# baycom/tfrec

Measured on AMD Instinct MI355X. Metric: IQ MSamples/s through demod+decode (batched streams), higher is better.
Workload: dtype int32+f32+f64

## Files before the change

### tfrec_amd/csrc/slicers.h

```cpp
#pragma once


struct Slicer {
	int lbi;
	int cur_block;
	int mark_lvl, rssi_i;
	int bitcnt, dmin, dmax, offset, last_bit;
	int first_cand_g;
	int td_lo, td_hi;
	int ib;
	int split;
	int hi, lo;
};
__device__ __forceinline__ void tfa2_thresholds(Slicer &f)
{
	const int noffset = d2i(0.9 * f.offset);
	f.hi = noffset + f.dmax / 32;
	f.lo = noffset + f.dmin / 32;
}

__device__ __forceinline__ void slicer_fresh(Slicer &f, int kind)
{
	f.mark_lvl = 0;
	f.rssi_i = 0;
	f.bitcnt = 0;
	f.dmin = 32767;
	f.dmax = -32767;
	f.offset = 0;
	f.last_bit = 0;
	f.first_cand_g = -1;
	f.hi = f.lo = 0;
	(void)kind;
}

__device__ __forceinline__ void slicer_chunk_begin(Slicer &f, int gf)
{
	const int b = gf >> 13;
	if (b != f.cur_block) {
		f.lbi = rebase_lbi(f.lbi, f.cur_block, b);
		f.cur_block = b;
	}
	const int o = gf & (kBlockDec - 1);
	f.ib = 2 * o;
	f.split = kBlockDec - o;
}
__device__ __forceinline__ int slicer_index(Slicer &f, int k)
{
	if (__builtin_expect(__ballot(k == f.split) != 0ull, 0)) {
		if (k == f.split) {
			f.lbi = rebase_lbi(f.lbi, f.cur_block, f.cur_block + 1);
			f.cur_block++;
			f.ib -= kIndexSpan;
		}
	}
	return f.ib + 2 * k;
}

__device__ __forceinline__ void tfa1_sample(Slicer &f, BitWriter &bw, int k, int I, int Q, int pI, int pQ)
{
	const int index = slicer_index(f, k);
	const int dev = fm_dev_nrzs(I, Q, pI, pQ);
	{
		const int decayed = tfa1_decay(f.mark_lvl);
		f.mark_lvl = dev > f.mark_lvl ? dev : decayed;
	}
	if (f.mark_lvl > f.rssi_i)
		f.rssi_i = f.mark_lvl;
	if (dev < (int)((uint32_t)f.mark_lvl >> 1)) {
		if (f.lbi) {
			const int gap = index - f.lbi;
			if (gap > 4) {
				for (int n = 22; n <= gap; n += 20)
					bw.put(1);
				bw.put(0);
			}
		}
		if (index - f.lbi > 2)
			f.lbi = index;
	}
}

__device__ __forceinline__ void tfa2_candidate(Slicer &f, BitWriter &bw, int g, int index, int bit, double spb, uint64_t nb_mul)
{
	if (f.first_cand_g < 0)
		f.first_cand_g = g;
	if (index > f.lbi + 8) {
		f.bitcnt++;
		const int tdiff = index - f.lbi;
		if (tdiff >= f.td_lo && tdiff <= f.td_hi) {
			const int numbits = nb_mul ? tfa2_numbits_mul(tdiff, nb_mul) : d2i(((tdiff / 2) + (spb / 2)) / spb);
			const int run = (numbits < 32 && numbits > 1) ? numbits - 1 : 0;
			bw.put_bits((f.last_bit ? (1u << run) - 1u : 0u) | ((uint32_t)bit << run), run + 1);
			f.last_bit = bit;
		}
	}
	if (index - f.lbi > 2)
		f.lbi = index;
}

__device__ __forceinline__ void tfa2_sample(Slicer &f, BitWriter &bw, int g, int k, int ld, uint32_t iq, double spb, uint64_t nb_mul)
{
	const int index = slicer_index(f, k);
	if (f.bitcnt < 10) {
		const bool up = ld > f.dmax, down = ld < f.dmin;
		if (up)
			f.dmax = (7 * f.dmax + ld) / 8;
		if (down)
			f.dmin = (7 * f.dmin + ld) / 8;
		if (up || down) {
			f.offset = (f.dmax + f.dmin) / 2;
			tfa2_thresholds(f);
		}
		if (f.bitcnt > 4) {
			const int I = (int)(int16_t)(iq & 0xffff), Q = (int)iq >> 16;
			const uint32_t t = (uint32_t)f.rssi_i + (uint32_t)(I * I) + (uint32_t)(Q * Q);
			f.rssi_i = (int)((uint32_t)f.rssi_i + (uint32_t)((int)t / 100));
		}
	}
	const int hi = f.hi, lo = f.lo;
	const int bit = ld > hi ? 1 : 0;
	if ((ld > hi || ld < lo) && bit != f.last_bit)
		tfa2_candidate(f, bw, g, index, bit, spb, nb_mul);
}

struct Slot8 {
	uint4 q0, q1, q2, q3, q4, q5, q6, q7;
};
struct Slot4 {
	uint4 q0, q1, q2, q3;
};

template <int KIND>
__device__ __forceinline__ int run_window(Slicer &f, BitWriter &bw, int g0, int last, bool closed,
					  const uint32_t *__restrict__ drow, const uint32_t *__restrict__ ldslots, int prevI,
					  int prevQ, double spb, uint64_t nb_mul, uint4 *__restrict__ my_lds, int head_chunks)
{
	const int n = last - g0 + 1;
	const int nch = (n + kChunk - 1) >> 5;
	if (KIND == 0) {
		auto load = [&](int i) -> Slot8 {
			const u32x4_a4 *p = reinterpret_cast<const u32x4_a4 *>(drow + g0 + kChunk * i);
			Slot8 r;
			u32x4_a4 v;
			v = p[0]; r.q0 = make_uint4(v.x, v.y, v.z, v.w);
			v = p[1]; r.q1 = make_uint4(v.x, v.y, v.z, v.w);
			v = p[2]; r.q2 = make_uint4(v.x, v.y, v.z, v.w);
			v = p[3]; r.q3 = make_uint4(v.x, v.y, v.z, v.w);
			v = p[4]; r.q4 = make_uint4(v.x, v.y, v.z, v.w);
			v = p[5]; r.q5 = make_uint4(v.x, v.y, v.z, v.w);
			v = p[6]; r.q6 = make_uint4(v.x, v.y, v.z, v.w);
			v = p[7]; r.q7 = make_uint4(v.x, v.y, v.z, v.w);
			return r;
		};
		int pI = prevI, pQ = prevQ;
		if (g0 > 0) {
			const uint32_t pw = drow[g0 - 1];
			pI = (int)(int16_t)(pw & 0xffff);
			pQ = (int)pw >> 16;
		}
		Slot8 cur = load(0);
		for (int i = 0; i < nch; i++) {
			my_lds[0 * 64] = cur.q0; my_lds[1 * 64] = cur.q1; my_lds[2 * 64] = cur.q2; my_lds[3 * 64] = cur.q3;
			my_lds[4 * 64] = cur.q4; my_lds[5 * 64] = cur.q5; my_lds[6 * 64] = cur.q6; my_lds[7 * 64] = cur.q7;
			const Slot8 nxt = load(i + 1 < nch ? i + 1 : i);
			const int nv = n - kChunk * i < kChunk ? n - kChunk * i : kChunk;
			slicer_chunk_begin(f, g0 + kChunk * i);
			uint4 vn = my_lds[0];
#pragma unroll 1
			for (int q = 0; 4 * q < nv; q++) {
				const uint4 v = vn;
				vn = my_lds[((q + 1) & 7) * 64];
				const uint32_t vw[4] = { v.x, v.y, v.z, v.w };
#pragma unroll
				for (int t = 0; t < 4; t++) {
					const int I = (int)(int16_t)(vw[t] & 0xffff), Q = (int)vw[t] >> 16;
					if (4 * q + t < nv)
						tfa1_sample(f, bw, 4 * q + t, I, Q, pI, pQ);
					pI = I;
					pQ = Q;
				}
			}
			bw.chunk_end();
			cur = nxt;
		}
	} else {
		auto load = [&](int i) -> Slot4 {
			const uint4 *p = reinterpret_cast<const uint4 *>(ldslots + (size_t)i * 16);
			Slot4 r;
			r.q0 = p[0]; r.q1 = p[1]; r.q2 = p[2]; r.q3 = p[3];
			return r;
		};
		Slot4 cur = load(0);
		for (int i = 0; i < nch; i++) {
			my_lds[0 * 64] = cur.q0; my_lds[1 * 64] = cur.q1; my_lds[2 * 64] = cur.q2; my_lds[3 * 64] = cur.q3;
			const Slot4 nxt = load(i + 1 < nch ? i + 1 : i);
			const int nv = n - kChunk * i < kChunk ? n - kChunk * i : kChunk;
			slicer_chunk_begin(f, g0 + kChunk * i);
			uint4 vn = my_lds[0];
#pragma unroll 1
			for (int q = 0; 8 * q < nv; q++) {
				const uint4 v = vn;
				vn = my_lds[((q + 1) & 3) * 64];
				const uint32_t vw[4] = { v.x, v.y, v.z, v.w };
#pragma unroll
				for (int t = 0; t < 8; t++) {
					if (8 * q + t < nv) {
						const int ld = (int)(int16_t)((vw[t >> 1] >> (16 * (t & 1))) & 0xffff);
						const uint32_t iq = (f.bitcnt > 4 && f.bitcnt < 10) ? drow[g0 + kChunk * i + 8 * q + t] : 0u;
						tfa2_sample(f, bw, g0 + kChunk * i + 8 * q + t, 8 * q + t, ld, iq, spb, nb_mul);
					}
				}
			}
			bw.chunk_end();
			cur = nxt;
			if (head_chunks > 0 && (f.bitcnt >= 10 || i + 1 >= head_chunks) && i + 1 < nch)
				return i + 1;
		}
	}
	const int bl = last >> 13;
	if (bl != f.cur_block) {
		f.lbi = rebase_lbi(f.lbi, f.cur_block, bl);
		f.cur_block = bl;
	}
	if (closed && KIND == 1)
		for (int q = 0; q < 16; q++)
			bw.put(f.last_bit);
	return nch;
}

template <int KIND>
__device__ __forceinline__ void window_task(int c, int j, int n_streams, int M, const uint32_t *__restrict__ dec,
					    size_t dec_stride, const int16_t *__restrict__ ld16, const ChainLaunch &L,
					    const WinTables &T, bool exact_lbi, int lbi_in_override, uint4 *__restrict__ my_lds,
					    int head_chunks)
{
	const int a = c / n_streams, s = c - a * n_streams;
	const ChainParams &p = L.params[a];
	const ChainState &st = L.states[a][s];
	const int og = T.open[(size_t)c * T.cap + j];
	const int close = T.close[(size_t)c * T.cap + j];
	const bool closed = close < M;
	const int last = closed ? close : M - 1;
	const bool cont = (j == 0) && T.cont[c];
	Slicer f;
	slicer_fresh(f, KIND);
	f.cur_block = og >> 13;
	if (cont) {
		f.mark_lvl = st.mark_lvl;
		f.rssi_i = st.rssi_i;
		f.bitcnt = st.bitcnt;
		f.dmin = st.dmin;
		f.dmax = st.dmax;
		f.offset = st.offset;
		f.last_bit = st.last_bit;
		f.lbi = rebase_lbi(st.last_bit_idx, -1, f.cur_block);
	} else if (KIND == 0) {
		f.lbi = 0;
	} else if (exact_lbi) {
		f.lbi = lbi_in_override;
	} else if (j == 0) {
		f.lbi = rebase_lbi(st.last_bit_idx, -1, f.cur_block);
	} else {
		f.lbi = kSpecLbi;
	}
	if (KIND == 1) {
		tfa2_thresholds(f);
		f.td_lo = (int)floor(p.spb / 4) + 1;
		f.td_hi = (int)ceil(32 * p.spb) - 1;
	}
	BitWriter bw{ T.bits + (size_t)c * T.bit_words + (og >> 6) + 3 * j, 0u, 0, 0u, -1 };
	const uint32_t *drow = dec + (size_t)s * dec_stride;
	const uint32_t *ldslots = (KIND == 1) ? reinterpret_cast<const uint32_t *>(ld16 + (size_t)(c - T.ld_c0) * T.slots * 32) +
							(size_t)win_slot0(og, j) * 16
					      : nullptr;
	const int resume = run_window<KIND>(f, bw, og, last, closed, drow, ldslots, st.prev_i, st.prev_q, p.spb, p.nb_mul, my_lds,
					    head_chunks);
	bw.finish();
	WinResult &r = T.result[(size_t)c * T.cap + j];
	r.resume = resume < ((last - og + 1 + kChunk - 1) >> 5) ? resume : -1;
	r.nbits = bw.n;
	r.closed = closed ? 1 : 0;
	r.rssi_i = f.rssi_i;
	r.offset = f.offset;
	r.lbi_out = f.lbi;
	r.first_cand_g = f.first_cand_g;
	r.bitcnt = f.bitcnt;
	r.dmin = f.dmin;
	r.dmax = f.dmax;
	r.last_bit = f.last_bit;
	r.mark_lvl = f.mark_lvl;
}

__global__ __launch_bounds__(64) void slicer_kernel(const uint32_t *__restrict__ dec, size_t dec_stride,
						    const int16_t *__restrict__ ld16, int n_streams, int n_blocks, ChainLaunch L,
						    WinTables T, int lanes, int head_chunks, int kind, int qsel)
{
	extern __shared__ uint4 slot_lds[];
	uint4 *my_lds = slot_lds + threadIdx.x;
	if ((int)threadIdx.x >= lanes)
		return;
	const int M = n_blocks * kBlockDec;
	const size_t total = (size_t)L.n_active * n_streams * T.cap;
	for (int q = 2 * kind + (kind == 0 ? 1 : 0); q < 2 * kind + 2; q++) {
		if ((qsel == 1 && (q & 1)) || (qsel == 2 && !(q & 1)))
			continue;
		const uint32_t count = T.queue[q].count;
		const int head = (q & 1) == 0 ? head_chunks : 0;
		while (true) {
			const uint32_t idx = atomicAdd(&T.queue[q].head, 1u);
			if (idx >= count)
				break;
			const uint2 it = T.items[(size_t)q * total + idx];
			const int c = (int)it.x, j = (int)it.y;
			if (kind == 0)
				window_task<0>(c, j, n_streams, M, dec, dec_stride, ld16, L, T, false, 0, my_lds, 0);
			else
				window_task<1>(c, j, n_streams, M, dec, dec_stride, ld16, L, T, false, 0, my_lds, head);
		}
	}
}

__global__ __launch_bounds__(256) void mark_kernel(const uint32_t *__restrict__ dec, size_t dec_stride, int n_streams,
						  int n_blocks, ChainLaunch L, WinTables T)
{
	const int M = n_blocks * kBlockDec;
	const size_t total = (size_t)L.n_active * n_streams * T.cap;
	const uint32_t count = T.queue[7].count;
	const uint32_t tid = blockIdx.x * 256 + threadIdx.x, nthreads = gridDim.x * 256;
	for (uint32_t idx = tid; idx < count; idx += nthreads) {
		const uint2 it = T.items[(size_t)7 * total + idx];
		const int c = (int)it.x, j = (int)(it.y & 0x1ffffu), pc = (int)(it.y >> 17);
		const int a = c / n_streams, s = c - a * n_streams;
		const ChainState &st = L.states[a][s];
		const int og = T.open[(size_t)c * T.cap + j];
		const int close = T.close[(size_t)c * T.cap + j];
		const int n = (close < M ? close : M - 1) - og + 1;
		const uint32_t *drow = dec + (size_t)s * dec_stride;
		const uint32_t prev0 = ((uint32_t)st.prev_i & 0xffffu) | ((uint32_t)st.prev_q << 16);
		const int slot0 = win_slot0(og, j);
		const int i0 = pc * kMarkSlots;
		const int nch = (n + 31) >> 5;
		const int i1 = nch < i0 + kMarkSlots ? nch : i0 + kMarkSlots;
		const int iw = pc == 0 ? 0 : i0 - kMarkWarmSlots;
		int mark = (pc == 0 && j == 0 && T.cont[c]) ? st.mark_lvl : 0;
		int start = mark, mx = 0;
		K3Chunk<true> A, B;
		k3_load<true>(A, drow, og + 32 * iw, prev0);
		for (int i = iw; i < i1; i++) {
			if (i + 1 < i1)
				k3_load<true>(B, drow, og + 32 * (i + 1), prev0);
			if (i == i0)
				start = mark;
			const int nv = n - 32 * i < 32 ? n - 32 * i : 32;
			int pI = (int)(int16_t)(A.prevw & 0xffff), pQ = (int)A.prevw >> 16;
			uint32_t bits = 0;
			if (__ballot(nv < 32) == 0ull) {
				uint32_t rev = 0;
				int dmax = -0x7fffffff;
#pragma unroll
				for (int k = 0; k < 32; k++) {
					const int I = (int)(int16_t)(A.w[k] & 0xffff), Q = (int)A.w[k] >> 16;
					const int dev = fm_dev_nrzs(I, Q, pI, pQ);
					const int decayed = tfa1_decay(mark);
					mark = dev > mark ? dev : decayed;
					const int half = (int)((uint32_t)mark >> 1);
					asm("v_cmp_lt_i32 vcc, %1, %2\n\tv_addc_co_u32 %0, vcc, %0, %0, vcc" : "+v"(rev) : "v"(dev), "v"(half) : "vcc");
					if (k == 0)
						mx = mark > mx ? mark : mx;
					else
						dmax = dev > dmax ? dev : dmax;
					pI = I;
					pQ = Q;
				}
				mx = dmax > mx ? dmax : mx;
				bits = __builtin_bitreverse32(rev);
			} else {
#pragma unroll
				for (int k = 0; k < 32; k++) {
					const int I = (int)(int16_t)(A.w[k] & 0xffff), Q = (int)A.w[k] >> 16;
					if (k < nv) {
						const int dev = fm_dev_nrzs(I, Q, pI, pQ);
						mark = dev > mark ? dev : tfa1_decay(mark);
						mx = mark > mx ? mark : mx;
						bits |= (uint32_t)(dev < mark / 2) << k;
					}
					pI = I;
					pQ = Q;
				}
			}
			if (i >= i0)
				T.cand[(size_t)s * T.slots + slot0 + i] = bits;
			else
				mx = 0;
			A = B;
		}
		MarkPiece mp;
		mp.start = start;
		mp.end = mark;
		mp.max = mx;
		mp.pad_ = 0;
		T.mark[(size_t)s * T.slots + slot0 + i0] = mp;
	}
}
```

Baseline: 305,100.

## Defer TFA2 RSSI accumulation out of the per-sample slicer loop into a span pass

Removes the conditional per-sample global load of raw IQ and the divide-based RSSI update from the TFA2 slicer's hot loop. Instead, the slicer records the sample indices where bitcnt reaches 5 and 10. A separate vectorized pass then walks only that span, eight samples per group, when the window ends or returns early. This cuts branchy scattered loads and register pressure in the main loop, at the cost of a second pass over the span and extra Slicer state. A Python model script checks that the deferred span matches the per-sample order, including across split windows.

```diff
diff --git a/profiles/ubench/tfa2_rssi_model.py b/profiles/ubench/tfa2_rssi_model.py
--- /dev/null
+++ b/profiles/ubench/tfa2_rssi_model.py
@@ -0,0 +1,99 @@
+#!/usr/bin/env python3
+import random
+import sys
+
+OPEN = 0x7FFFFFFF
+
+
+def u32(x):
+    return x & 0xFFFFFFFF
+
+
+def i32(x):
+    x &= 0xFFFFFFFF
+    return x - (1 << 32) if x & 0x80000000 else x
+
+
+def cdiv(a, b):
+    q = abs(a) // abs(b)
+    return q if (a >= 0) == (b >= 0) else -q
+
+
+def rssi_step(rssi, iq):
+    I, Q = iq
+    t = u32(u32(rssi) + u32(I * I) + u32(Q * Q))
+    return i32(u32(rssi) + u32(cdiv(i32(t), 100)))
+
+
+def per_sample(row, cand, g0, n, bitcnt, rssi):
+    for g in range(g0, g0 + n):
+        if 4 < bitcnt < 10:
+            rssi = rssi_step(rssi, row[g])
+        if cand[g]:
+            bitcnt += 1
+    return bitcnt, rssi
+
+
+def rssi_span(rssi, row, beg, end, loads=None):
+    if beg >= end:
+        return rssi
+    g = beg & ~7
+    while g < end:
+        assert g + 8 <= len(row), "a group leaves the row"
+        if loads is not None:
+            loads.append(g)
+        for t in range(8):
+            if beg <= g + t < end:
+                rssi = rssi_step(rssi, row[g + t])
+        g += 8
+    return rssi
+
+
+def peeled(row, cand, g0, n, bitcnt, rssi, loads=None):
+    rs_beg = g0 if bitcnt > 4 else OPEN
+    rs_end = g0 if bitcnt >= 10 else OPEN
+    for g in range(g0, g0 + n):
+        if cand[g]:
+            bitcnt += 1
+            rs_beg = g + 1 if bitcnt == 5 else rs_beg
+            rs_end = g + 1 if bitcnt == 10 else rs_end
+    walked_end = g0 + n
+    rssi = rssi_span(rssi, row, rs_beg, min(rs_end, walked_end), loads)
+    return bitcnt, rssi
+
+
+def random_window(rng, big=False):
+    m = 8 * rng.randrange(8, 40)
+    lim = 32767 if big else rng.choice((40, 2000, 32767))
+    row = [(rng.randint(-lim - 1, lim), rng.randint(-lim - 1, lim)) for _ in range(m)]
+    dens = rng.choice((0.0, 0.02, 0.1, 0.5))
+    cand = [rng.random() < dens for _ in range(m)]
+    g0 = rng.randrange(0, m // 2)
+    n = rng.randrange(1, m - g0 + 1)
+    return row, cand, g0, n
+
+
+def main():
+    seed = int(sys.argv[1]) if len(sys.argv) > 1 else 1
+    trials = int(sys.argv[2]) if len(sys.argv) > 2 else 2000
+    rng = random.Random(seed)
+    splits = summed = 0
+    for _ in range(trials):
+        row, cand, g0, n = random_window(rng)
+        b0 = rng.choice((0, 0, 3, 4, 5, 7, 9, 10, 12))
+        r0 = i32(rng.getrandbits(32)) if b0 > 4 else 0
+        want = per_sample(row, cand, g0, n, b0, r0)
+        loads = []
+        assert peeled(row, cand, g0, n, b0, r0, loads) == want
+        summed += len(loads)
+        if n > 1:
+            k = rng.randrange(1, n)
+            mid = peeled(row, cand, g0, k, b0, r0)
+            assert mid == per_sample(row, cand, g0, k, b0, r0)
+            assert peeled(row, cand, g0 + k, n - k, *mid) == want
+            splits += 1
+    print("ok: %d windows, %d with a split, %d groups summed" % (trials, splits, summed))
+
+
+if __name__ == "__main__":
+    main()
diff --git a/tfrec_amd/csrc/slicers.h b/tfrec_amd/csrc/slicers.h
--- a/tfrec_amd/csrc/slicers.h
+++ b/tfrec_amd/csrc/slicers.h
@@ -11,7 +11,9 @@
 	int ib;
 	int split;
 	int hi, lo;
+	int rs_beg, rs_end;
 };
+constexpr int kRsOpen = 0x7fffffff;
 __device__ __forceinline__ void tfa2_thresholds(Slicer &f)
 {
 	const int noffset = d2i(0.9 * f.offset);
@@ -86,6 +88,8 @@
 		f.first_cand_g = g;
 	if (index > f.lbi + 8) {
 		f.bitcnt++;
+		f.rs_beg = f.bitcnt == 5 ? g + 1 : f.rs_beg;
+		f.rs_end = f.bitcnt == 10 ? g + 1 : f.rs_end;
 		const int tdiff = index - f.lbi;
 		if (tdiff >= f.td_lo && tdiff <= f.td_hi) {
 			const int numbits = nb_mul ? tfa2_numbits_mul(tdiff, nb_mul) : d2i(((tdiff / 2) + (spb / 2)) / spb);
@@ -98,7 +102,7 @@
 		f.lbi = index;
 }
 
-__device__ __forceinline__ void tfa2_sample(Slicer &f, BitWriter &bw, int g, int k, int ld, uint32_t iq, double spb, uint64_t nb_mul)
+__device__ __forceinline__ void tfa2_sample(Slicer &f, BitWriter &bw, int g, int k, int ld, double spb, uint64_t nb_mul)
 {
 	const int index = slicer_index(f, k);
 	if (f.bitcnt < 10) {
@@ -111,11 +115,6 @@
 			f.offset = (f.dmax + f.dmin) / 2;
 			tfa2_thresholds(f);
 		}
-		if (f.bitcnt > 4) {
-			const int I = (int)(int16_t)(iq & 0xffff), Q = (int)iq >> 16;
-			const uint32_t t = (uint32_t)f.rssi_i + (uint32_t)(I * I) + (uint32_t)(Q * Q);
-			f.rssi_i = (int)((uint32_t)f.rssi_i + (uint32_t)((int)t / 100));
-		}
 	}
 	const int hi = f.hi, lo = f.lo;
 	const int bit = ld > hi ? 1 : 0;
@@ -129,6 +128,40 @@
 struct Slot4 {
 	uint4 q0, q1, q2, q3;
 };
+
+struct Slot2 {
+	uint4 q0, q1;
+};
+__device__ __forceinline__ int tfa2_rssi_span(int rssi, const uint32_t *__restrict__ drow, int beg, int end)
+{
+	if (beg >= end)
+		return rssi;
+	auto load = [&](int g) -> Slot2 {
+		const u32x4_a4 *p = reinterpret_cast<const u32x4_a4 *>(drow + g);
+		Slot2 r;
+		u32x4_a4 v;
+		v = p[0]; r.q0 = make_uint4(v.x, v.y, v.z, v.w);
+		v = p[1]; r.q1 = make_uint4(v.x, v.y, v.z, v.w);
+		return r;
+	};
+	int g = beg & ~7;
+	Slot2 nx = load(g);
+#pragma unroll 1
+	for (; g < end; g += 8) {
+		const Slot2 v = nx;
+		if (g + 8 < end)
+			nx = load(g + 8);
+		const uint32_t vw[8] = { v.q0.x, v.q0.y, v.q0.z, v.q0.w, v.q1.x, v.q1.y, v.q1.z, v.q1.w };
+#pragma unroll
+		for (int t = 0; t < 8; t++) {
+			const int I = (int)(int16_t)(vw[t] & 0xffff), Q = (int)vw[t] >> 16;
+			const uint32_t u = (uint32_t)rssi + (uint32_t)(I * I) + (uint32_t)(Q * Q);
+			const int r = (int)((uint32_t)rssi + (uint32_t)((int)u / 100));
+			rssi = (g + t >= beg && g + t < end) ? r : rssi;
+		}
+	}
+	return rssi;
+}
 
 template <int KIND>
 __device__ __forceinline__ int run_window(Slicer &f, BitWriter &bw, int g0, int last, bool closed,
@@ -190,6 +223,11 @@
 			r.q0 = p[0]; r.q1 = p[1]; r.q2 = p[2]; r.q3 = p[3];
 			return r;
 		};
+		f.rs_beg = f.bitcnt > 4 ? g0 : kRsOpen;
+		f.rs_end = f.bitcnt >= 10 ? g0 : kRsOpen;
+		auto rssi_behind = [&](int walked_end) {
+			f.rssi_i = tfa2_rssi_span(f.rssi_i, drow, f.rs_beg, f.rs_end < walked_end ? f.rs_end : walked_end);
+		};
 		Slot4 cur = load(0);
 		for (int i = 0; i < nch; i++) {
 			my_lds[0 * 64] = cur.q0; my_lds[1 * 64] = cur.q1; my_lds[2 * 64] = cur.q2; my_lds[3 * 64] = cur.q3;
@@ -206,16 +244,18 @@
 				for (int t = 0; t < 8; t++) {
 					if (8 * q + t < nv) {
 						const int ld = (int)(int16_t)((vw[t >> 1] >> (16 * (t & 1))) & 0xffff);
-						const uint32_t iq = (f.bitcnt > 4 && f.bitcnt < 10) ? drow[g0 + kChunk * i + 8 * q + t] : 0u;
-						tfa2_sample(f, bw, g0 + kChunk * i + 8 * q + t, 8 * q + t, ld, iq, spb, nb_mul);
+						tfa2_sample(f, bw, g0 + kChunk * i + 8 * q + t, 8 * q + t, ld, spb, nb_mul);
 					}
 				}
 			}
 			bw.chunk_end();
 			cur = nxt;
-			if (head_chunks > 0 && (f.bitcnt >= 10 || i + 1 >= head_chunks) && i + 1 < nch)
+			if (head_chunks > 0 && (f.bitcnt >= 10 || i + 1 >= head_chunks) && i + 1 < nch) {
+				rssi_behind(g0 + kChunk * (i + 1));
 				return i + 1;
-		}
+			}
+		}
+		rssi_behind(last + 1);
 	}
 	const int bl = last >> 13;
 	if (bl != f.cur_block) {
```

New measurement: 307,800, median of 6. Within noise of the previous version (+0.9%).
